# OpenSLAM-org/openslam_g2o

Hardware: AMD Instinct MI355X
Metric: linear-solve ms/iter (buildSystem + setLambda + solve + restoreDiagonal), 100k-pose BA (lower is better)
Workload: dtype f64; 1 GPU; synthetic BA (BASELINE.json configs[3]): 100000 poses / 1000000 landmarks / 5000000 observations, BlockSolver_6_3 semantics, Schur + multifrontal block Cholesky, lambda=10; poses=100000, landmarks=1000000, edges=5000000, parallelism=1 GPU, edge_data=estimates+measurements in HBM, errors/Jacobians evaluated inside buildSystem, information=identity, declared for the whole edge set (not read per edge)

## Files before the change

include/g2ohip.h:

```cpp
#ifndef G2OHIP_H
#define G2OHIP_H

#include <stddef.h>
#include <stdint.h>

#ifdef __cplusplus
extern "C" {
#endif

#define G2OHIP_OK 0
#define G2OHIP_NOT_PD 1
#define G2OHIP_REPEAT 2
#define G2OHIP_ERR_ARG (-1)
#define G2OHIP_ERR_HIP (-2)
#define G2OHIP_ERR_STATE (-3)
#define G2OHIP_ERR_UNSUPPORTED (-4)

#define G2OHIP_KERNEL_NONE 0
#define G2OHIP_KERNEL_HUBER 1
#define G2OHIP_KERNEL_PSEUDOHUBER 2
#define G2OHIP_KERNEL_CAUCHY 3
#define G2OHIP_KERNEL_SATURATED 4
#define G2OHIP_KERNEL_DCS 5

// ... 130 lines not shown
int g2ohip_solve_reduced(g2ohip_solver* s);
int g2ohip_solve_back_substitute(g2ohip_solver* s);

int g2ohip_host_register(g2ohip_solver* s, void* ptr, size_t bytes);
int g2ohip_host_unregister(g2ohip_solver* s, void* ptr);

int g2ohip_ba_set_edges(g2ohip_solver* s, int set, const int32_t* cam_vertex, const int32_t* point_vertex, const double* meas,
                        const double* info, double focal_length, double cx, double cy);
int g2ohip_ba_set_edges_classes(g2ohip_solver* s, int set, const int32_t* cam_vertex, const int32_t* point_vertex, const double* meas,
                                const double* info, int n_classes, const double* class_params, const int32_t* edge_class);
int g2ohip_ba_set_estimates(g2ohip_solver* s, int n_cams, const double* cams, const int32_t* cam_hidx, int n_points,
                            const double* points, const int32_t* point_hidx);
int g2ohip_ba_get_estimates(g2ohip_solver* s, double* cams, double* points);
int g2ohip_ba_get_estimates_of(g2ohip_solver* s, int n_cams, const int32_t* cam_index, double* cams, int n_points, const int32_t* point_index,
                               double* points);
int g2ohip_ba_fetch_estimates_begin(g2ohip_solver* s, double* cams, double* points, int point_pieces);
int g2ohip_ba_fetch_estimates_wait(g2ohip_solver* s, int piece);
int g2ohip_ba_linearize(g2ohip_solver* s, int jacobians);
int g2ohip_ba_update(g2ohip_solver* s);
int g2ohip_ba_push(g2ohip_solver* s);
int g2ohip_ba_pop(g2ohip_solver* s);
int g2ohip_ba_discard_top(g2ohip_solver* s);

int g2ohip_pg_set_edges(g2ohip_solver* s, int set, int type, const int32_t* vi, const int32_t* vj, const double* meas,
                        const double* info);
int g2ohip_pg_set_estimates(g2ohip_solver* s, int n_vertices, const double* poses, const int32_t* hidx);
int g2ohip_pg_get_estimates(g2ohip_solver* s, double* poses);
int g2ohip_pg_linearize(g2ohip_solver* s, int jacobians);
int g2ohip_pg_update(g2ohip_solver* s);
int g2ohip_pg_push(g2ohip_solver* s);
// ... 24 lines not shown
```

openslam_g2o_amd/capi.py:

```python
import ctypes as C
import os
import sys

import numpy as np

_HERE = os.path.dirname(os.path.abspath(__file__))
LIB_PATH = os.environ.get("G2OHIP_LIB") or os.path.join(_HERE, "lib", "libg2ohip.so")

c_int_p = C.POINTER(C.c_int32)
c_dbl_p = C.POINTER(C.c_double)

OK, NOT_PD, REPEAT = 0, 1, 2
ERR_UNSUPPORTED = -4
HPP, HPL, HLL, HSCHUR, DINV = 0, 1, 2, 3, 4
PART_NO_VERTEX0, PART_NO_VERTEX1, PART_NO_CHI2 = 1, 2, 4
ARR_BSCHUR, ARR_X, ARR_B, ARR_EXCHANGE, ARR_XP, ARR_XBOUNDARY, ARR_XHALO, ARR_SCHUR_DIAG = 100, 101, 102, 103, 104, 105, 106, 107
KERNEL_NONE, KERNEL_HUBER, KERNEL_PSEUDOHUBER, KERNEL_CAUCHY, KERNEL_SATURATED, KERNEL_DCS = 0, 1, 2, 3, 4, 5


class Stats(C.Structure):
    _fields_ = [(n, C.c_double) for n in (
        "timeQuadraticForm", "timeSchurComplement", "timeSymbolicDecomposition", "timeNumericDecomposition",
        "timeLinearSolution", "timeLinearSolver", "timeBackSubstitution")] + [(n, C.c_size_t) for n in (
            "hessianDimension", "hessianPoseDimension", "hessianLandmarkDimension", "choleskyNNZ", "numFronts",
# ... 2 lines not shown

    def as_dict(self):
        return {n: getattr(self, n) for n, _ in self._fields_}


EXPORTS = [
    "g2ohip_last_error", "g2ohip_device_count", "g2ohip_create", "g2ohip_destroy", "g2ohip_set_stream", "g2ohip_init",
    "g2ohip_add_edge_set", "g2ohip_build_structure", "g2ohip_set_edge_data", "g2ohip_set_edge_errors", "g2ohip_set_robust_kernel", "g2ohip_set_robust_kernel_per_edge",
    "g2ohip_build_system", "g2ohip_chi2", "g2ohip_set_lambda", "g2ohip_restore_diagonal", "g2ohip_max_diagonal",
    "g2ohip_compute_scale", "g2ohip_solve", "g2ohip_vector_size", "g2ohip_copy_x", "g2ohip_copy_b", "g2ohip_x_device",
    "g2ohip_b_device", "g2ohip_multiply_hessian", "g2ohip_sync", "g2ohip_set_profiling", "g2ohip_get_stats",
    "g2ohip_set_option", "g2ohip_get_nnzb", "g2ohip_get_pattern", "g2ohip_copy_values", "g2ohip_device_array",
    "g2ohip_solve_schur", "g2ohip_solve_reduced", "g2ohip_solve_back_substitute", "g2ohip_ls_create",
    "g2ohip_ls_destroy", "g2ohip_ls_init", "g2ohip_ls_solve", "g2ohip_ls_solve_pattern", "g2ohip_ls_get_stats", "g2ohip_ls_set_option",
    "g2ohip_kernel_slots", "g2ohip_kernel_name", "g2ohip_kernel_time", "g2ohip_add_schur_pattern", "g2ohip_set_edge_set_parts",
    "g2ohip_set_lambda_split", "g2ohip_host_register", "g2ohip_host_unregister", "g2ohip_ba_set_edges", "g2ohip_ba_set_edges_classes", "g2ohip_ba_set_estimates", "g2ohip_ba_get_estimates", "g2ohip_ba_get_estimates_of", "g2ohip_ba_fetch_estimates_begin", "g2ohip_ba_fetch_estimates_wait",
    "g2ohip_ba_linearize", "g2ohip_ba_update", "g2ohip_ba_push", "g2ohip_ba_pop", "g2ohip_ba_discard_top",
    "g2ohip_set_partition", "g2ohip_solve_reduced_local", "g2ohip_solve_reduced_shared", "g2ohip_solve_reduced_finish",
    "g2ohip_schur_operator_prepare", "g2ohip_schur_operator_apply", "g2ohip_solve_async", "g2ohip_trial_stats_begin", "g2ohip_trial_stats", "g2ohip_solve_reduced_finish_async", "g2ohip_exchange_setup", "g2ohip_exchange_pack", "g2ohip_exchange_unpack", "g2ohip_exchange_status",
    "g2ohip_get_partition", "g2ohip_partition_poses",
    "g2ohip_pg_set_edges", "g2ohip_pg_set_estimates", "g2ohip_pg_get_estimates", "g2ohip_pg_linearize", "g2ohip_pg_update",
    "g2ohip_pg_push", "g2ohip_pg_pop", "g2ohip_pg_discard_top", "g2ohip_copy_edge_data",
    "g2ohip_pg_set_landmark_edges", "g2ohip_pg_set_landmark_estimates", "g2ohip_pg_get_landmark_estimates",
    "g2ohip_compute_marginals", "g2ohip_set_x", "g2ohip_copy_diagonal",
    "g2ohip_comm_unique_id", "g2ohip_comm_init_rccl", "g2ohip_comm_init_host", "g2ohip_comm_init_peer", "g2ohip_comm_destroy", "g2ohip_comm_all_reduce",
    "g2ohip_update_structure", "g2ohip_clear_edge_sets", "g2ohip_solve_sharded", "g2ohip_chi2_sharded", "g2ohip_max_diagonal_sharded", "g2ohip_compute_scale_sharded",
]

HOST_ALLREDUCE_FN = C.CFUNCTYPE(C.c_int, C.c_void_p, C.POINTER(C.c_double), C.c_size_t, C.c_int)

_lib = None
# ... 61 lines not shown
    L.g2ohip_set_profiling.argtypes = [vp, C.c_int]
    L.g2ohip_get_stats.argtypes = [vp, C.POINTER(Stats)]
    L.g2ohip_set_option.argtypes = [vp, C.c_char_p, C.c_double]
    L.g2ohip_get_nnzb.argtypes = [vp, C.c_int, C.POINTER(C.c_int)]
    L.g2ohip_get_pattern.argtypes = [vp, C.c_int, c_int_p, c_int_p]
    L.g2ohip_copy_values.argtypes = [vp, C.c_int, c_dbl_p]
    L.g2ohip_device_array.argtypes = [vp, C.c_int, C.POINTER(vp), C.POINTER(C.c_size_t)]
    L.g2ohip_add_schur_pattern.argtypes = [vp, C.c_int, c_int_p, c_int_p]
    L.g2ohip_set_edge_set_parts.argtypes = [vp, C.c_int, C.c_int]
    L.g2ohip_set_lambda_split.argtypes = [vp, C.c_double, C.c_double, C.c_int]
    L.g2ohip_ba_set_edges.argtypes = [vp, C.c_int, c_int_p, c_int_p, c_dbl_p, c_dbl_p, C.c_double, C.c_double, C.c_double]
    L.g2ohip_ba_set_edges_classes.argtypes = [vp, C.c_int, c_int_p, c_int_p, c_dbl_p, c_dbl_p, C.c_int, c_dbl_p, c_int_p]
    L.g2ohip_ba_set_estimates.argtypes = [vp, C.c_int, c_dbl_p, c_int_p, C.c_int, c_dbl_p, c_int_p]
    L.g2ohip_ba_get_estimates.argtypes = [vp, c_dbl_p, c_dbl_p]
    L.g2ohip_ba_get_estimates_of.argtypes = [vp, C.c_int, c_int_p, c_dbl_p, C.c_int, c_int_p, c_dbl_p]
    L.g2ohip_set_edge_errors.argtypes = [vp, C.c_int, c_dbl_p]
    L.g2ohip_ba_fetch_estimates_begin.argtypes = [vp, c_dbl_p, c_dbl_p, C.c_int]
    L.g2ohip_ba_fetch_estimates_wait.argtypes = [vp, C.c_int]
    L.g2ohip_ba_linearize.argtypes = [vp, C.c_int]
    for n in ("g2ohip_ba_update", "g2ohip_ba_push", "g2ohip_ba_pop", "g2ohip_ba_discard_top", "g2ohip_pg_update", "g2ohip_pg_push",
              "g2ohip_pg_pop", "g2ohip_pg_discard_top"):
        getattr(L, n).argtypes = [vp]
    L.g2ohip_pg_set_edges.argtypes = [vp, C.c_int, C.c_int, c_int_p, c_int_p, c_dbl_p, c_dbl_p]
    L.g2ohip_pg_set_estimates.argtypes = [vp, C.c_int, c_dbl_p, c_int_p]
    L.g2ohip_pg_get_estimates.argtypes = [vp, c_dbl_p]
    L.g2ohip_pg_linearize.argtypes = [vp, C.c_int]
    L.g2ohip_pg_set_landmark_edges.argtypes = [vp, C.c_int, C.c_int, c_int_p, c_int_p, c_dbl_p, c_dbl_p, c_dbl_p]
    L.g2ohip_pg_set_landmark_estimates.argtypes = [vp, C.c_int, c_dbl_p, c_int_p]
    L.g2ohip_pg_get_landmark_estimates.argtypes = [vp, c_dbl_p]
    L.g2ohip_copy_edge_data.argtypes = [vp, C.c_int, c_dbl_p, c_dbl_p, c_dbl_p]
# ... 47 lines not shown
    return a.ctypes.data_as(c_dbl_p)


def _ptr(a):
    if a is None:
        return None, None
    if isinstance(a, np.ndarray):
        return C.c_void_p(a.ctypes.data), False
    if isinstance(a, int):
        return C.c_void_p(a), True
    if hasattr(a, "data_ptr"):
        return C.c_void_p(a.data_ptr()), bool(a.is_cuda)
    raise TypeError(type(a))


class HipBlockSolver:

    def __init__(self, pose_dim, landmark_dim, device=0):
        self.L = load()
        self.p, self.l = pose_dim, landmark_dim
        self.h = C.c_void_p()
        _check(self.L.g2ohip_create(C.byref(self.h), pose_dim, landmark_dim, device), "g2ohip_create")
        self._keep = {}
        self.nP = self.nL = 0

    def close(self):
        if getattr(self, "h", None) is not None and self.h.value:
            self.L.g2ohip_destroy(self.h)
            self.h = C.c_void_p()

# ... 317 lines not shown
        _check(self.L.g2ohip_ba_set_estimates(self.h, len(ch), _dp(cams), _ip(ch), len(ph), _dp(points), _ip(ph)),
               "baSetEstimates")

    def baGetEstimates(self):
        cams = np.empty((self._ba_n[0], 12))
        pts = np.empty((self._ba_n[1], 3))
        _check(self.L.g2ohip_ba_get_estimates(self.h, _dp(cams), _dp(pts)), "baGetEstimates")
        return cams, pts

    def baGetEstimatesOf(self, cam_index, point_index):
        ci, pi = _i32(cam_index), _i32(point_index)
        cams, pts = np.empty((len(ci), 12)), np.empty((len(pi), 3))
        _check(self.L.g2ohip_ba_get_estimates_of(self.h, len(ci), _ip(ci), _dp(cams), len(pi), _ip(pi), _dp(pts)), "baGetEstimatesOf")
        return cams, pts

    def baFetchEstimatesBegin(self, pieces=4):
        self._fetch = (np.empty((self._ba_n[0], 12)), np.empty((self._ba_n[1], 3)), pieces)
        _check(self.L.g2ohip_ba_fetch_estimates_begin(self.h, _dp(self._fetch[0]), _dp(self._fetch[1]), pieces), "baFetchEstimatesBegin")

    def baFetchEstimatesWait(self, piece):
        _check(self.L.g2ohip_ba_fetch_estimates_wait(self.h, piece), "baFetchEstimatesWait")
        return self._fetch[0], self._fetch[1]

    def baLinearize(self, jacobians=True):
        _check(self.L.g2ohip_ba_linearize(self.h, int(jacobians)), "baLinearize")

    def baUpdate(self):
        _check(self.L.g2ohip_ba_update(self.h), "baUpdate")

    def baPush(self):
# ... 183 lines not shown
```

openslam_g2o_amd/csrc/block_solver.h:

```cpp
#pragma once
#include <memory>

#include "common.h"
#include "comm.h"
#include "block_pcg.h"
#include "sparse_cholesky.h"

namespace g2ohip {

struct EdgeSet {
  int d = 0, n = 0, dim0 = 0, dim1 = 0;
  bool unary = false;
  int parts = 0;
  std::vector<int> v0, v1;
  int kernel_kind = 0;
  double delta = 1.0;
  DevBuf<double> rk;
  const double *J0 = nullptr, *J1 = nullptr, *omega = nullptr, *err = nullptr;
  DevBuf<double> own_J0, own_J1, own_omega, own_err;
  bool has_data = false;
  bool external = false;
  bool has_err = false;
  DevBuf<int> vp_ptr, vp_ent, vl_ptr, vl_ent;
  DevBuf<int> vp_act;
  int n_vp_act = 0;
  std::vector<int> h_vp_ent, h_vl_ent;
  std::vector<int> h_vl_ptr;
  DevBuf<int> op_dst, op_ptr, op_ent;
  DevBuf<int> ol_dst, ol_ptr, ol_ent;
  int n_op = 0, n_ol = 0;
  long n_vp_ent = 0, n_vl_ent = 0;
  bool touches_pose = false, touches_lm = false, first_pose = false, first_lm = false, first_op = false, first_ol = false;
};

struct SolverTimes {
  double quadratic = 0, schur = 0, numeric = 0, linsolve = 0, backsub = 0, residuals = 0, linearize = 0, update = 0;
};

class BlockSolver {
 public:
  BlockSolver(int p, int l, int device);
  ~BlockSolver();

  void init();
  void clear_edge_sets();
  int add_edge_set(int d, int n, const int* v0, const int* v1);
  void set_edge_set_parts(int set, int parts);
  void add_schur_pattern(int n, const int* rows, const int* cols);
  void build_structure(int nP, int nL, bool do_schur);
  bool update_structure(int new_poses, int set, int n, const int* v0, const int* v1);
  void set_edge_data(int set, const double* J0, const double* J1, const double* omega, const double* err, bool on_device);
  void set_edge_errors(int set, const double* err);
// ... 44 lines not shown
  void sync();
  void set_stream(hipStream_t st);
  hipStream_t stream() const { return st_; }

  int nnzb(int which) const;
  void get_pattern(int which, int* colptr, int* rowidx) const;
  void copy_values(int which, double* h);
  void device_array(int which, double** ptr, size_t* count);

  void ba_set_edges(int set, const int* cam_vertex, const int* point_vertex, const double* meas, const double* info, double f,
                    double cx, double cy);
  void ba_set_edges_classes(int set, const int* cam_vertex, const int* point_vertex, const double* meas, const double* info, double f,
                            double cx, double cy, int n_classes, const double* class_params, const int* edge_class);
  void ba_set_estimates(int n_cams, const double* cams, const int* cam_hidx, int n_points, const double* points, const int* point_hidx);
  void ba_get_estimates(double* cams, double* points);
  void ba_get_estimates_of(int n_cams, const int* cam_idx, double* cams, int n_points, const int* point_idx, double* points);
  void ba_fetch_begin(double* cams, double* points, int point_pieces);
  void ba_fetch_wait(int piece);
  static constexpr int kFetchMaxPieces = 17;
  void ba_linearize(bool jacobians);
  void ba_update();
  void ba_push();
  void ba_pop();
  void ba_discard_top();

  bool profiling = false;
  KernelProf prof;
  SolverTimes times;
  CholOptions chol_opt;
  size_t schur_tile_bytes = 39 * 1024;
// ... 180 lines not shown
    bool err_valid = false, jac_valid = false;
    DevBuf<double> chi_part;
    bool fused_ok = false;
    DevBuf<double> meas, cams, pts, cams_bak, pts_bak;
    DevBuf<double> meas_pm, omega_pm;
    DevBuf<int> pt_pm, cam_pm;
    DevBuf<double> meas_lm, omega_lm;
    DevBuf<int> cam_q, pt_q;
    DevBuf<double> meas_q, omega_q;
    DevBuf<int> cam_lm, pt_lm, hpl_lm, row_lm;
    DevBuf<int4> ll_rec;
    DevBuf<int> ll_edge;
    DevBuf<int> ll_row;
    DevBuf<double> ll_meas, ll_omega;
    DevBuf<int4> tile_ll;
    DevBuf<int> sel_idx;
    DevBuf<double> sel_out;
    bool ll_slots_ok = false;
    bool has_backup = false;
  } ba_;
  struct PgFrontEnd {
    int set = -1, type = 0, nv = 0;
    DevBuf<int> vi, vj, hidx;
    std::vector<int> h_vi, h_vj, h_hidx;
    DevBuf<double> meas, poses, poses_bak;
    bool has_backup = false;
    bool err_valid = false, jac_valid = false;
    int lm_set = -1, lm_type = 0, n_points = 0;
    DevBuf<int> vp, vl, pt_hidx;
    std::vector<int> h_vp, h_vl, h_pt_hidx;
// ... 10 lines not shown
```

openslam_g2o_amd/csrc/block_solver.hip:

```cpp
#include "block_solver.h"

#include <algorithm>
#include <atomic>
#include <chrono>
#include <cmath>
#include <cstring>
#include <numeric>

namespace g2ohip {

namespace {

constexpr int kThreads = 256;

template <int CTRL>
__device__ __forceinline__ double dpp_permute(double v) {
  const int lo = __double2loint(v), hi = __double2hiint(v);
  const int lo2 = __builtin_amdgcn_update_dpp(lo, lo, CTRL, 0xf, 0xf, true);
  const int hi2 = __builtin_amdgcn_update_dpp(hi, hi, CTRL, 0xf, 0xf, true);
  return __hiloint2double(hi2, lo2);
}
template <int G>
__device__ __forceinline__ double group_sum(double v) {
  if (G >= 2) v += dpp_permute<0xB1>(v);
// ... 1408 lines not shown
  if (!active || g >= 3) return;
  double cl[3];
#pragma unroll
  for (int j = 0; j < 3; ++j) cl[j] = c[j] + bl[(size_t)lm * 3 + j];
  const double* D = Dinv + (size_t)lm * 9;
  if (G == 1) {
#pragma unroll
    for (int i = 0; i < 3; ++i) xl[(size_t)lm * 3 + i] = D[i] * cl[0] + D[i + 3] * cl[1] + D[i + 6] * cl[2];
  } else {
    xl[(size_t)lm * 3 + g] = D[g] * cl[0] + D[g + 3] * cl[1] + D[g + 6] * cl[2];
  }
}

template <bool CLS>
__global__ void __launch_bounds__(kThreads) ba_back_substitute_slots_kernel(
    const int* __restrict__ tile_lm0, const int4* __restrict__ tile_ll, const int4* __restrict__ ll_rec, const int* __restrict__ ll_row,
    const double* __restrict__ ll_meas, const double* __restrict__ ll_omega, const double* __restrict__ cams,
    const double* __restrict__ pts, double f, double cx, double cy, int kind, double delta, int ident, const double* __restrict__ Dinv,
    const double* __restrict__ bl, const double* __restrict__ xp, double* __restrict__ xl, const double* __restrict__ ctab) {
  const int t = blockIdx.x, tid = threadIdx.x, NT = blockDim.x;
  const int l0 = tile_lm0[(size_t)t * 8];
  const int4 tl = tile_ll[t];
  for (int sb = 0; sb < tl.y; sb += NT) {
    const int si = sb + tid;
    const size_t sg = (size_t)tl.x + min(si, tl.y - 1);
    int4 rc = ll_rec[sg];
    if (si >= tl.y) rc.x = (int)0x80000fffu;
    const int ent = rc.x;
    const int krel = ent & 0xfff, K = (ent >> 12) & 0xff, lmi = (ent >> 20) & 0x7ff;
    const bool head = ent >= 0;
    const int pos = head ? 0 : lmi;
    const int row = krel != 0xfff ? ll_row[sg] : -1;
    double c[3] = {0.0, 0.0, 0.0};
    {
      double T[12], X[3], z2[2], Op[4], xv[6];
      const double* Xp = pts + (size_t)rc.z * 3;
      X[0] = Xp[0]; X[1] = Xp[1]; X[2] = Xp[2];
      load_vec<12>(cams + (size_t)ba_edge_class<CLS>(rc.y, ctab, f, cx, cy, kind, delta) * 12, T);
      load_vec<2>(ll_meas + sg * 2, z2);
      load_vec<6>(xp + (size_t)max(row, 0) * 6, xv);
      if (ident) {
        Op[0] = Op[3] = 1.0;
        Op[1] = Op[2] = 0.0;
      } else {
        load_vec<4>(ll_omega + sg * 4, Op);
      }
      if (row >= 0) {
        BaEdgeLin L;
        ba_edge_linearize(T, X, z2, Op, f, cx, cy, kind, delta, true, L);
        double t0 = 0.0, t1 = 0.0;
#pragma unroll
        for (int a = 0; a < 6; ++a) {
          t0 += L.B[0 + 2 * a] * xv[a];
          t1 += L.B[1 + 2 * a] * xv[a];
        }
        const double w = L.w;
        const double u0 = w * (L.O[0] * t0 + L.O[2] * t1), u1 = w * (L.O[1] * t0 + L.O[3] * t1);
#pragma unroll
        for (int j = 0; j < 3; ++j) c[j] = -(L.A[0 + 2 * j] * u0 + L.A[1 + 2 * j] * u1);
      }
    }
    for (int d = 1; d < tl.w; d <<= 1) {
      const bool take = pos + d < K;
#pragma unroll
      for (int i = 0; i < 3; ++i) {
        const double o = __shfl_down(c[i], d);
        if (take) c[i] += o;
      }
    }
    if (head) {
      const int lm = l0 + lmi;
      double cl[3];
#pragma unroll
      for (int j = 0; j < 3; ++j) cl[j] = c[j] + bl[(size_t)lm * 3 + j];
      const double* D = Dinv + (size_t)lm * 9;
#pragma unroll
      for (int i = 0; i < 3; ++i) xl[(size_t)lm * 3 + i] = D[i] * cl[0] + D[i + 3] * cl[1] + D[i + 6] * cl[2];
    }
  }
}

#ifndef G2OHIP_ASMP_OCC
#define G2OHIP_ASMP_OCC 2
#endif
template <int G, bool CLS = false>
__global__ void __launch_bounds__(kThreads, G2OHIP_ASMP_OCC) ba_assemble_poses_kernel(
    int nP, const int* __restrict__ vptr, const double* __restrict__ cams, const double* __restrict__ pts,
    const int* __restrict__ cam_pm, const int* __restrict__ pt_pm, const double* __restrict__ meas_pm, const double* __restrict__ omega_pm,
    double f, double cx, double cy, int kind, double delta, double* __restrict__ Hpp, const int* __restrict__ diag_blk,
    double* __restrict__ bp, int accumulate, int ident, const int* __restrict__ act, const double* __restrict__ ctab) {
  const int gt = blockIdx.x * blockDim.x + threadIdx.x;
  const int vi_ = gt / G, g = gt % G;
  const bool active = vi_ < nP;
// ... 2431 lines not shown

void BlockSolver::solve_back_substitute() {
  require_structure();
  if (!schur_) return;
  G2OHIP_HIP_CHECK(hipSetDevice(device_));
  solve_back_substitute_impl();
}

void BlockSolver::solve_back_substitute_impl() {
  if (profiling) tb_.start(st_);
  const size_t sizeP = (size_t)nP_ * p_;
  prof.begin(KernelProf::kBackSub, st_);
  if (ba_recompute_ok()) {
    EdgeSet& es = *sets_[ba_.set];
    const int GL = ba_lm_group();
    if (ba_fuse_landmarks && ba_.ll_slots_ok && n_tiles_ > 0) {
#define G2OHIP_BA_BACK_SLOTS(CC)                                                                                                   \
  hipLaunchKernelGGL((ba_back_substitute_slots_kernel<CC>), dim3(n_tiles_), dim3(kThreads), 0, st_, d_tile_lm0.p, ba_.tile_ll.p,    \
                     ba_.ll_rec.p, ba_.ll_row.p, ba_.ll_meas.p, ba_.ll_omega.p, ba_.cams.p, ba_.pts.p, ba_.f, ba_.cx, ba_.cy,       \
                     es.kernel_kind, es.delta, ba_.omega_identity ? 1 : 0, d_Dinv.p, d_b.p + sizeP, d_x.p, d_x.p + sizeP, ba_.ctab.p)
      if (ba_.n_classes > 1) G2OHIP_BA_BACK_SLOTS(true);
      else G2OHIP_BA_BACK_SLOTS(false);
#undef G2OHIP_BA_BACK_SLOTS
    } else
#define G2OHIP_BA_BACK(GG) G2OHIP_BA_BACK_(GG, false)
#define G2OHIP_BA_BACK_(GG, CC)                                                                                                    \
  hipLaunchKernelGGL((ba_back_substitute_kernel<GG, CC>), dim3(grid_for((size_t)nL_ * GG)), dim3(kThreads), 0, st_, nL_, es.vl_ptr.p, \
                     ba_.cams.p, ba_.pts.p, ba_.cam_lm.p, ba_.pt_lm.p, ba_.meas_lm.p, ba_.omega_lm.p, ba_.row_lm.p, ba_.f,          \
                     ba_.cx, ba_.cy, es.kernel_kind, es.delta, ba_.omega_identity ? 1 : 0, d_Dinv.p, d_b.p + sizeP, d_x.p,           \
                     d_x.p + sizeP, ba_.ctab.p)
    if (ba_.n_classes > 1) G2OHIP_BA_BACK_(8, true);
    else if (GL == 1) G2OHIP_BA_BACK(1);
    else if (GL == 4) G2OHIP_BA_BACK(4);
    else G2OHIP_BA_BACK(8);
#undef G2OHIP_BA_BACK
// ... 441 lines not shown
  const size_t k = (size_t)blockIdx.x * blockDim.x + threadIdx.x;
  if (k >= n) return;
  const size_t e = (size_t)(ent[k] >> 1);
  cam_o[k] = cam_v[e];
  pt_o[k] = pt_v[e];
  meas_o[2 * k] = meas[2 * e];
  meas_o[2 * k + 1] = meas[2 * e + 1];
  if (omega_o)
    for (int i = 0; i < 4; ++i) omega_o[4 * k + i] = omega[4 * e + i];
  if (hpl_o) {
    const int h = edge_hpl[e];
    hpl_o[k] = h;
    row_o[k] = h >= 0 ? v1[e] : -1;
  }
}
__global__ void ba_gather_slots_kernel(const int4* __restrict__ tile_ll, const int* __restrict__ slots, const int* __restrict__ vl_ent,
                                       const int* __restrict__ cam_lm, const int* __restrict__ pt_lm, const int* __restrict__ hpl_lm,
                                       const int* __restrict__ row_lm, const double* __restrict__ meas_lm, const double* __restrict__ omega_lm,
                                       int4* __restrict__ rec, int* __restrict__ edge, int* __restrict__ srow, double* __restrict__ ms,
                                       double* __restrict__ os) {
  const int4 tl = tile_ll[blockIdx.x];
  for (int i = threadIdx.x; i < tl.y; i += blockDim.x) {
    const size_t sidx = (size_t)tl.x + i;
    const int w = slots[sidx];
    int4 r = make_int4(w, 0, 0, -1);
    int ed = 0, row = -1;
    double m0 = 0.0, m1 = 0.0, o[4] = {0.0, 0.0, 0.0, 0.0};
    if ((w & 0xfff) != 0xfff) {
      const size_t k = (size_t)tl.z + (w & 0xfff);
      r = make_int4(w, cam_lm[k], pt_lm[k], hpl_lm[k]);
// ... 140 lines not shown
    ba_.meas_lm.alloc(std::max<size_t>(nl * 2, 1));
    ba_.cam_lm.alloc(std::max<size_t>(nl, 1));
    ba_.pt_lm.alloc(std::max<size_t>(nl, 1));
    ba_.hpl_lm.alloc(std::max<size_t>(nl, 1));
    ba_.row_lm.alloc(std::max<size_t>(nl, 1));
    if (d_omega) ba_.omega_lm.alloc(std::max<size_t>(nl * 4, 1));
    if (nl)
      hipLaunchKernelGGL(ba_gather_lists_kernel, dim3(grid_for(nl)), dim3(kThreads), 0, st_, nl, es.vl_ent.p, ba_.cam_v.p, ba_.pt_v.p, ba_.meas.p,
                         d_omega, ba_.edge_hpl.p, d_v1.p, ba_.cam_lm.p, ba_.pt_lm.p, ba_.meas_lm.p,
                         d_omega ? ba_.omega_lm.p : (double*)nullptr, ba_.hpl_lm.p, ba_.row_lm.p);
    G2OHIP_HIP_CHECK(hipGetLastError());
    lap("pose-major + landmark-major copies");
    ba_.ll_slots_ok = false;
    if (schur_ && n_tiles_ > 0 && tiles_cover_all_ && n_split_tiles_ == 0 && (int)tile_lm0_h_.size() == n_tiles_ + 1 &&
        (int)es.h_vl_ptr.size() == nL_ + 1) {
      constexpr int kIdleSlot = (int)0x80000fffu;
      std::vector<int4> tl((size_t)n_tiles_);
      std::vector<int> cnt((size_t)n_tiles_, 0);
      std::atomic<bool> okf(true);
      auto walk = [&](int t, int* out, int& kmax) {
        const int l0 = tile_lm0_h_[t], l1 = tile_lm0_h_[t + 1];
        const int kb = es.h_vl_ptr[l0];
        int used = 0, total = 0;
        kmax = 0;
        for (int lm = l0; lm < l1; ++lm) {
          const int K = es.h_vl_ptr[lm + 1] - es.h_vl_ptr[lm], lmi = lm - l0;
          if (K > 64 || lmi >= 0x7ff || es.h_vl_ptr[lm + 1] - kb >= 0xfff) return -1;
          const int need = std::max(K, 1);
          if (used + need > 64) {
            if (out)
              for (int i = used; i < 64; ++i) out[total + i - used] = kIdleSlot;
            total += 64 - used;
            used = 0;
          }
          if (out) {
            if (K == 0) out[total] = 0xfff | (lmi << 20);
            for (int j = 0; j < K; ++j)
              out[total + j] = (es.h_vl_ptr[lm] + j - kb) | (K << 12) | (j == 0 ? (lmi << 20) : (int)(0x80000000u | ((unsigned)j << 20)));
          }
          total += need;
          used = (used + need) & 63;
          kmax = std::max(kmax, K);
        }
        if (used) {
          if (out)
            for (int i = used; i < 64; ++i) out[total + i - used] = kIdleSlot;
          total += 64 - used;
        }
        return total;
      };
      host_parallel_for((size_t)n_tiles_, [&](size_t t0_, size_t t1_) {
        for (size_t t = t0_; t < t1_; ++t) {
          int kmax = 0;
          const int c = walk((int)t, nullptr, kmax);
          if (c < 0) okf.store(false);
          cnt[t] = std::max(c, 0);
        }
      }, 64);
      size_t ns = 0;
      for (int t = 0; t < n_tiles_; ++t) {
        tl[t].x = (int)ns;
        ns += (size_t)cnt[t];
      }
      if (okf.load() && ns < ((size_t)1 << 31)) {
        std::vector<int> slots(std::max<size_t>(ns, 1), kIdleSlot);
        host_parallel_for((size_t)n_tiles_, [&](size_t t0_, size_t t1_) {
          for (size_t t = t0_; t < t1_; ++t) {
            int kmax = 0;
            walk((int)t, slots.data() + tl[t].x, kmax);
            tl[t] = make_int4(tl[t].x, cnt[t], es.h_vl_ptr[tile_lm0_h_[t]], kmax);
          }
        }, 64);
        const size_t nsa = slots.size();
        DevBuf<int> d_slots;
        d_slots.upload(slots, st_);
        ba_.tile_ll.upload(tl, st_);
        ba_.ll_rec.alloc(nsa);
        ba_.ll_edge.alloc(nsa);
        ba_.ll_row.alloc(nsa);
        ba_.ll_meas.alloc(nsa * 2);
        if (d_omega) ba_.ll_omega.alloc(nsa * 4);
        if (ns == 0) {
          const int4 idle = make_int4(kIdleSlot, 0, 0, -1);
          const int none = -1;
          ba_.ll_rec.upload(&idle, 1, st_);
          ba_.ll_row.upload(&none, 1, st_);
          ba_.ll_edge.zero(st_);
          ba_.ll_meas.zero(st_);
        } else {
          hipLaunchKernelGGL(ba_gather_slots_kernel, dim3(n_tiles_), dim3(kThreads), 0, st_, ba_.tile_ll.p, d_slots.p, es.vl_ent.p, ba_.cam_lm.p,
                             ba_.pt_lm.p, ba_.hpl_lm.p, ba_.row_lm.p, ba_.meas_lm.p, d_omega ? ba_.omega_lm.p : (const double*)nullptr,
// ... 6 lines not shown
    }
    lap("lane slots of the tiles");
    G2OHIP_HIP_CHECK(hipStreamSynchronize(st_));
  }
  lap("pose-major / landmark-major uploads");
  if (!(ba_fused && ba_.fused_ok)) {
    es.own_J0.alloc(n * 6);
    es.own_J1.alloc(n * 12);
  }
  es.own_err.alloc(n * 2);
  es.J0 = es.own_J0.p; es.J1 = es.own_J1.p; es.omega = es.own_omega.p; es.err = es.own_err.p;
  es.has_data = false;
  prepare_ba_tile_kernels();
  G2OHIP_HIP_CHECK(hipStreamSynchronize(st_));
  lap("buffers, kernel attributes, sync");
}

bool BlockSolver::ba_recompute_ok() const {
  if (!schur_ || p_ != 6 || l_ != 3 || ba_.set < 0 || !ba_fused || !ba_.fused_ok || ba_.n_cams <= 0) return false;
  if (ba_.sys_version < 0 || ba_.sys_version != ba_.est_version) return false;
  const EdgeSet& bs = *sets_[ba_.set];
  if (bs.kernel_kind != ba_.sys_kind || bs.delta != ba_.sys_delta) return false;
  for (size_t i = 0; i < sets_.size(); ++i)
    if ((int)i != ba_.set && sets_[i]->n > 0 && sets_[i]->touches_lm) return false;
  return true;
}

void BlockSolver::ba_validate() {
  if (ba_.set < 0 || ba_.h_cam_v.empty() || ba_.h_cam_hidx.empty()) return;
  ba_validate_edges(*sets_[ba_.set], ba_.h_cam_v.data(), ba_.h_pt_v.data(), ba_.h_cam_v.size());
// ... 643 lines not shown
```

openslam_g2o_amd/csrc/capi.hip:

```cpp
#include "../../include/g2ohip.h"

#include <cstdlib>
#include <cstring>
#include <string>

#include "block_solver.h"

namespace g2ohip {
std::string& last_error_ref() {
  static thread_local std::string e;
  return e;
}
}

using namespace g2ohip;

struct g2ohip_solver {
  std::unique_ptr<BlockSolver> impl;
};

struct g2ohip_linear_solver {
  int bs = 0, device = 0;
  hipStream_t st = nullptr;
  std::unique_ptr<SparseCholesky> chol;
// ... 631 lines not shown
int g2ohip_ba_get_estimates(g2ohip_solver* s, double* cams, double* points) {
  REQUIRE_HANDLE(s);
  return guarded([&] {
    s->impl->ba_get_estimates(cams, points);
    return G2OHIP_OK;
  });
}
int g2ohip_ba_get_estimates_of(g2ohip_solver* s, int n_cams, const int32_t* cam_index, double* cams, int n_points, const int32_t* point_index,
                               double* points) {
  REQUIRE_HANDLE(s);
  return guarded([&] {
    s->impl->ba_get_estimates_of(n_cams, cam_index, cams, n_points, point_index, points);
    return G2OHIP_OK;
  });
}
int g2ohip_ba_fetch_estimates_begin(g2ohip_solver* s, double* cams, double* points, int point_pieces) {
  REQUIRE_HANDLE(s);
  return guarded([&] {
    s->impl->ba_fetch_begin(cams, points, point_pieces);
    return G2OHIP_OK;
  });
}
int g2ohip_ba_fetch_estimates_wait(g2ohip_solver* s, int piece) {
  REQUIRE_HANDLE(s);
  return guarded([&] {
    s->impl->ba_fetch_wait(piece);
    return G2OHIP_OK;
  });
}
int g2ohip_ba_linearize(g2ohip_solver* s, int jacobians) {
// ... 356 lines not shown
```

Before: 1.141 ms/iter.

## Run landmark back-substitution as persistent 64-lane groups with prefetch

```diff
diff --git a/include/g2ohip.h b/include/g2ohip.h
--- a/include/g2ohip.h
+++ b/include/g2ohip.h
@@ -168,6 +168,10 @@
 int g2ohip_ba_get_estimates(g2ohip_solver* s, double* cams, double* points);
 int g2ohip_ba_get_estimates_of(g2ohip_solver* s, int n_cams, const int32_t* cam_index, double* cams, int n_points, const int32_t* point_index,
                                double* points);
+int g2ohip_ba_plan_lane_slots(int n_tiles, const int32_t* tile_lm0, const int32_t* list_ptr, long long* n_slots, int32_t* tile_ll,
+                              int32_t* group_ll, int32_t* slot_words);
+int g2ohip_ba_get_lane_slots(g2ohip_solver* s, int* n_tiles, long long* n_slots, int32_t* tile_lm0, int32_t* tile_ll, int32_t* group_ll,
+                             int32_t* slot_words);
 int g2ohip_ba_fetch_estimates_begin(g2ohip_solver* s, double* cams, double* points, int point_pieces);
 int g2ohip_ba_fetch_estimates_wait(g2ohip_solver* s, int piece);
 int g2ohip_ba_linearize(g2ohip_solver* s, int jacobians);
diff --git a/openslam_g2o_amd/capi.py b/openslam_g2o_amd/capi.py
--- a/openslam_g2o_amd/capi.py
+++ b/openslam_g2o_amd/capi.py
@@ -40,7 +40,7 @@
     "g2ohip_solve_schur", "g2ohip_solve_reduced", "g2ohip_solve_back_substitute", "g2ohip_ls_create",
     "g2ohip_ls_destroy", "g2ohip_ls_init", "g2ohip_ls_solve", "g2ohip_ls_solve_pattern", "g2ohip_ls_get_stats", "g2ohip_ls_set_option",
     "g2ohip_kernel_slots", "g2ohip_kernel_name", "g2ohip_kernel_time", "g2ohip_add_schur_pattern", "g2ohip_set_edge_set_parts",
-    "g2ohip_set_lambda_split", "g2ohip_host_register", "g2ohip_host_unregister", "g2ohip_ba_set_edges", "g2ohip_ba_set_edges_classes", "g2ohip_ba_set_estimates", "g2ohip_ba_get_estimates", "g2ohip_ba_get_estimates_of", "g2ohip_ba_fetch_estimates_begin", "g2ohip_ba_fetch_estimates_wait",
+    "g2ohip_set_lambda_split", "g2ohip_host_register", "g2ohip_host_unregister", "g2ohip_ba_set_edges", "g2ohip_ba_set_edges_classes", "g2ohip_ba_set_estimates", "g2ohip_ba_get_estimates", "g2ohip_ba_get_estimates_of", "g2ohip_ba_plan_lane_slots", "g2ohip_ba_get_lane_slots", "g2ohip_ba_fetch_estimates_begin", "g2ohip_ba_fetch_estimates_wait",
     "g2ohip_ba_linearize", "g2ohip_ba_update", "g2ohip_ba_push", "g2ohip_ba_pop", "g2ohip_ba_discard_top",
     "g2ohip_set_partition", "g2ohip_solve_reduced_local", "g2ohip_solve_reduced_shared", "g2ohip_solve_reduced_finish",
     "g2ohip_schur_operator_prepare", "g2ohip_schur_operator_apply", "g2ohip_solve_async", "g2ohip_trial_stats_begin", "g2ohip_trial_stats", "g2ohip_solve_reduced_finish_async", "g2ohip_exchange_setup", "g2ohip_exchange_pack", "g2ohip_exchange_unpack", "g2ohip_exchange_status",
@@ -132,6 +132,8 @@
     L.g2ohip_ba_set_estimates.argtypes = [vp, C.c_int, c_dbl_p, c_int_p, C.c_int, c_dbl_p, c_int_p]
     L.g2ohip_ba_get_estimates.argtypes = [vp, c_dbl_p, c_dbl_p]
     L.g2ohip_ba_get_estimates_of.argtypes = [vp, C.c_int, c_int_p, c_dbl_p, C.c_int, c_int_p, c_dbl_p]
+    L.g2ohip_ba_plan_lane_slots.argtypes = [C.c_int, c_int_p, c_int_p, C.POINTER(C.c_longlong), c_int_p, c_int_p, c_int_p]
+    L.g2ohip_ba_get_lane_slots.argtypes = [vp, C.POINTER(C.c_int), C.POINTER(C.c_longlong), c_int_p, c_int_p, c_int_p, c_int_p]
     L.g2ohip_set_edge_errors.argtypes = [vp, C.c_int, c_dbl_p]
     L.g2ohip_ba_fetch_estimates_begin.argtypes = [vp, c_dbl_p, c_dbl_p, C.c_int]
     L.g2ohip_ba_fetch_estimates_wait.argtypes = [vp, C.c_int]
@@ -209,6 +211,20 @@
     raise TypeError(type(a))
 
 
+def plan_lane_slots(tile_lm0, list_ptr):
+    L = load()
+    tl0, lp = _i32(tile_lm0), _i32(list_ptr)
+    nt, ns = len(tl0) - 1, C.c_longlong()
+    _check(L.g2ohip_ba_plan_lane_slots(nt, _ip(tl0), _ip(lp), C.byref(ns), None, None, None), "plan_lane_slots")
+    if ns.value < 0:
+        return None
+    t = dict(tile_ll=np.zeros((nt, 4), dtype=np.int32), group_ll=np.zeros((ns.value // 64, 2), dtype=np.int32),
+             slot_words=np.zeros(ns.value, dtype=np.int32))
+    _check(L.g2ohip_ba_plan_lane_slots(nt, _ip(tl0), _ip(lp), C.byref(ns), _ip(t["tile_ll"]), _ip(t["group_ll"]), _ip(t["slot_words"])),
+           "plan_lane_slots")
+    return t
+
+
 class HipBlockSolver:
 
     def __init__(self, pose_dim, landmark_dim, device=0):
@@ -556,6 +572,15 @@
         _check(self.L.g2ohip_ba_get_estimates_of(self.h, len(ci), _ip(ci), _dp(cams), len(pi), _ip(pi), _dp(pts)), "baGetEstimatesOf")
         return cams, pts
 
+    def baLaneSlots(self):
+        nt, ns = C.c_int(), C.c_longlong()
+        _check(self.L.g2ohip_ba_get_lane_slots(self.h, C.byref(nt), C.byref(ns), None, None, None, None), "baLaneSlots")
+        t = dict(tile_lm0=np.zeros(nt.value + 1, dtype=np.int32), tile_ll=np.zeros((nt.value, 4), dtype=np.int32),
+                 group_ll=np.zeros((ns.value // 64, 2), dtype=np.int32), slot_words=np.zeros(ns.value, dtype=np.int32))
+        _check(self.L.g2ohip_ba_get_lane_slots(self.h, None, None, _ip(t["tile_lm0"]), _ip(t["tile_ll"]), _ip(t["group_ll"]),
+                                               _ip(t["slot_words"])), "baLaneSlots")
+        return t
+
     def baFetchEstimatesBegin(self, pieces=4):
         self._fetch = (np.empty((self._ba_n[0], 12)), np.empty((self._ba_n[1], 3)), pieces)
         _check(self.L.g2ohip_ba_fetch_estimates_begin(self.h, _dp(self._fetch[0]), _dp(self._fetch[1]), pieces), "baFetchEstimatesBegin")
diff --git a/openslam_g2o_amd/csrc/block_solver.h b/openslam_g2o_amd/csrc/block_solver.h
--- a/openslam_g2o_amd/csrc/block_solver.h
+++ b/openslam_g2o_amd/csrc/block_solver.h
@@ -36,6 +36,13 @@
 struct SolverTimes {
   double quadratic = 0, schur = 0, numeric = 0, linsolve = 0, backsub = 0, residuals = 0, linearize = 0, update = 0;
 };
+
+struct BaLaneSlots {
+  std::vector<int4> tile_ll;
+  std::vector<int> slots;
+  std::vector<int2> group_ll;
+};
+bool ba_plan_lane_slots(int n_tiles, const int* tile_lm0, const int* vl_ptr, BaLaneSlots& out);
 
 class BlockSolver {
  public:
@@ -110,6 +117,7 @@
                             double cx, double cy, int n_classes, const double* class_params, const int* edge_class);
   void ba_set_estimates(int n_cams, const double* cams, const int* cam_hidx, int n_points, const double* points, const int* point_hidx);
   void ba_get_estimates(double* cams, double* points);
+  void ba_get_lane_slots(int* n_tiles, long long* n_slots, int* tile_lm0, int* tile_ll, int* group_ll, int* slot_words);
   void ba_get_estimates_of(int n_cams, const int* cam_idx, double* cams, int n_points, const int* point_idx, double* points);
   void ba_fetch_begin(double* cams, double* points, int point_pieces);
   void ba_fetch_wait(int piece);
@@ -320,6 +328,11 @@
     DevBuf<int> ll_row;
     DevBuf<double> ll_meas, ll_omega;
     DevBuf<int4> tile_ll;
+    DevBuf<int2> group_ll;
+    int n_groups = 0;
+    int back_wg_per_cu[2] = {1, 1};
+    std::vector<int4> h_tile_ll;
+    std::vector<int2> h_group_ll;
     DevBuf<int> sel_idx;
     DevBuf<double> sel_out;
     bool ll_slots_ok = false;
diff --git a/openslam_g2o_amd/csrc/block_solver.hip b/openslam_g2o_amd/csrc/block_solver.hip
--- a/openslam_g2o_amd/csrc/block_solver.hip
+++ b/openslam_g2o_amd/csrc/block_solver.hip
@@ -1446,53 +1446,67 @@
 
 template <bool CLS>
 __global__ void __launch_bounds__(kThreads) ba_back_substitute_slots_kernel(
-    const int* __restrict__ tile_lm0, const int4* __restrict__ tile_ll, const int4* __restrict__ ll_rec, const int* __restrict__ ll_row,
+    int n_groups, const int2* __restrict__ group_ll, const int4* __restrict__ ll_rec, const int* __restrict__ ll_row,
     const double* __restrict__ ll_meas, const double* __restrict__ ll_omega, const double* __restrict__ cams,
     const double* __restrict__ pts, double f, double cx, double cy, int kind, double delta, int ident, const double* __restrict__ Dinv,
     const double* __restrict__ bl, const double* __restrict__ xp, double* __restrict__ xl, const double* __restrict__ ctab) {
-  const int t = blockIdx.x, tid = threadIdx.x, NT = blockDim.x;
-  const int l0 = tile_lm0[(size_t)t * 8];
-  const int4 tl = tile_ll[t];
-  for (int sb = 0; sb < tl.y; sb += NT) {
-    const int si = sb + tid;
-    const size_t sg = (size_t)tl.x + min(si, tl.y - 1);
-    int4 rc = ll_rec[sg];
-    if (si >= tl.y) rc.x = (int)0x80000fffu;
+  const int lane = threadIdx.x & 63, wpb = blockDim.x >> 6;
+  const int stride = gridDim.x * wpb;
+  int g = blockIdx.x * wpb + (threadIdx.x >> 6);
+  if (g >= n_groups) return;
+  size_t sg = (size_t)g * 64 + lane;
+  int4 rc = ll_rec[sg];
+  int row = ll_row[sg];
+  double z2[2];
+  load_vec<2>(ll_meas + sg * 2, z2);
+  int2 gl = group_ll[g];
+  for (;;) {
     const int ent = rc.x;
     const int krel = ent & 0xfff, K = (ent >> 12) & 0xff, lmi = (ent >> 20) & 0x7ff;
     const bool head = ent >= 0;
     const int pos = head ? 0 : lmi;
-    const int row = krel != 0xfff ? ll_row[sg] : -1;
+    if (krel == 0xfff) row = -1;
+    double T[12], X[3], Op[4], xv[6], blv[3], D[9];
+    const double* Xp = pts + (size_t)rc.z * 3;
+    X[0] = Xp[0]; X[1] = Xp[1]; X[2] = Xp[2];
+    load_vec<12>(cams + (size_t)ba_edge_class<CLS>(rc.y, ctab, f, cx, cy, kind, delta) * 12, T);
+    load_vec<6>(xp + (size_t)max(row, 0) * 6, xv);
+    if (ident) {
+      Op[0] = Op[3] = 1.0;
+      Op[1] = Op[2] = 0.0;
+    } else {
+      load_vec<4>(ll_omega + sg * 4, Op);
+    }
+    const int lm = gl.x + (head ? lmi : 0);
+#pragma unroll
+    for (int j = 0; j < 3; ++j) blv[j] = bl[(size_t)lm * 3 + j];
+#pragma unroll
+    for (int j = 0; j < 9; ++j) D[j] = Dinv[(size_t)lm * 9 + j];
+    const int gn = g + stride;
+    const bool more = gn < n_groups;
+    const int gq = more ? gn : g;
+    const size_t sn = (size_t)gq * 64 + lane;
+    const int4 rcn = ll_rec[sn];
+    const int rown = ll_row[sn];
+    double zn[2];
+    load_vec<2>(ll_meas + sn * 2, zn);
+    const int2 gln = group_ll[gq];
     double c[3] = {0.0, 0.0, 0.0};
-    {
-      double T[12], X[3], z2[2], Op[4], xv[6];
-      const double* Xp = pts + (size_t)rc.z * 3;
-      X[0] = Xp[0]; X[1] = Xp[1]; X[2] = Xp[2];
-      load_vec<12>(cams + (size_t)ba_edge_class<CLS>(rc.y, ctab, f, cx, cy, kind, delta) * 12, T);
-      load_vec<2>(ll_meas + sg * 2, z2);
-      load_vec<6>(xp + (size_t)max(row, 0) * 6, xv);
-      if (ident) {
-        Op[0] = Op[3] = 1.0;
-        Op[1] = Op[2] = 0.0;
-      } else {
-        load_vec<4>(ll_omega + sg * 4, Op);
+    if (row >= 0) {
+      BaEdgeLin L;
+      ba_edge_linearize(T, X, z2, Op, f, cx, cy, kind, delta, true, L);
+      double t0 = 0.0, t1 = 0.0;
+#pragma unroll
+      for (int a = 0; a < 6; ++a) {
+        t0 += L.B[0 + 2 * a] * xv[a];
+        t1 += L.B[1 + 2 * a] * xv[a];
       }
-      if (row >= 0) {
-        BaEdgeLin L;
-        ba_edge_linearize(T, X, z2, Op, f, cx, cy, kind, delta, true, L);
-        double t0 = 0.0, t1 = 0.0;
-#pragma unroll
-        for (int a = 0; a < 6; ++a) {
-          t0 += L.B[0 + 2 * a] * xv[a];
-          t1 += L.B[1 + 2 * a] * xv[a];
-        }
-        const double w = L.w;
-        const double u0 = w * (L.O[0] * t0 + L.O[2] * t1), u1 = w * (L.O[1] * t0 + L.O[3] * t1);
-#pragma unroll
-        for (int j = 0; j < 3; ++j) c[j] = -(L.A[0 + 2 * j] * u0 + L.A[1 + 2 * j] * u1);
-      }
-    }
-    for (int d = 1; d < tl.w; d <<= 1) {
+      const double w = L.w;
+      const double u0 = w * (L.O[0] * t0 + L.O[2] * t1), u1 = w * (L.O[1] * t0 + L.O[3] * t1);
+#pragma unroll
+      for (int j = 0; j < 3; ++j) c[j] = -(L.A[0 + 2 * j] * u0 + L.A[1 + 2 * j] * u1);
+    }
+    for (int d = 1; d < gl.y; d <<= 1) {
       const bool take = pos + d < K;
 #pragma unroll
       for (int i = 0; i < 3; ++i) {
@@ -1501,14 +1515,19 @@
       }
     }
     if (head) {
-      const int lm = l0 + lmi;
       double cl[3];
 #pragma unroll
-      for (int j = 0; j < 3; ++j) cl[j] = c[j] + bl[(size_t)lm * 3 + j];
-      const double* D = Dinv + (size_t)lm * 9;
+      for (int j = 0; j < 3; ++j) cl[j] = c[j] + blv[j];
 #pragma unroll
       for (int i = 0; i < 3; ++i) xl[(size_t)lm * 3 + i] = D[i] * cl[0] + D[i + 3] * cl[1] + D[i + 6] * cl[2];
     }
+    if (!more) break;
+    g = gn;
+    sg = sn;
+    rc = rcn;
+    row = rown;
+    z2[0] = zn[0]; z2[1] = zn[1];
+    gl = gln;
   }
 }
 
@@ -3970,11 +3989,13 @@
   if (ba_recompute_ok()) {
     EdgeSet& es = *sets_[ba_.set];
     const int GL = ba_lm_group();
-    if (ba_fuse_landmarks && ba_.ll_slots_ok && n_tiles_ > 0) {
+    if (ba_fuse_landmarks && ba_.ll_slots_ok && ba_.n_groups > 0) {
 #define G2OHIP_BA_BACK_SLOTS(CC)                                                                                                   \
-  hipLaunchKernelGGL((ba_back_substitute_slots_kernel<CC>), dim3(n_tiles_), dim3(kThreads), 0, st_, d_tile_lm0.p, ba_.tile_ll.p,    \
-                     ba_.ll_rec.p, ba_.ll_row.p, ba_.ll_meas.p, ba_.ll_omega.p, ba_.cams.p, ba_.pts.p, ba_.f, ba_.cx, ba_.cy,       \
-                     es.kernel_kind, es.delta, ba_.omega_identity ? 1 : 0, d_Dinv.p, d_b.p + sizeP, d_x.p, d_x.p + sizeP, ba_.ctab.p)
+  hipLaunchKernelGGL((ba_back_substitute_slots_kernel<CC>),                                                                        \
+                     dim3(std::min((ba_.n_groups + kThreads / 64 - 1) / (kThreads / 64), num_cus_ * ba_.back_wg_per_cu[CC])),      \
+                     dim3(kThreads), 0, st_, ba_.n_groups, ba_.group_ll.p, ba_.ll_rec.p, ba_.ll_row.p, ba_.ll_meas.p,               \
+                     ba_.ll_omega.p, ba_.cams.p, ba_.pts.p, ba_.f, ba_.cx, ba_.cy, es.kernel_kind, es.delta,                       \
+                     ba_.omega_identity ? 1 : 0, d_Dinv.p, d_b.p + sizeP, d_x.p, d_x.p + sizeP, ba_.ctab.p)
       if (ba_.n_classes > 1) G2OHIP_BA_BACK_SLOTS(true);
       else G2OHIP_BA_BACK_SLOTS(false);
 #undef G2OHIP_BA_BACK_SLOTS
@@ -4446,6 +4467,79 @@
     row_o[k] = h >= 0 ? v1[e] : -1;
   }
 }
+bool ba_plan_lane_slots(int n_tiles, const int* tile_lm0, const int* vl_ptr, BaLaneSlots& out) {
+  constexpr int kIdleSlot = (int)0x80000fffu;
+  std::vector<int4>& tl = out.tile_ll;
+  tl.assign((size_t)n_tiles, make_int4(0, 0, 0, 0));
+  out.slots.clear();
+  out.group_ll.clear();
+  std::vector<int> cnt((size_t)n_tiles, 0);
+  std::atomic<bool> okf(true);
+  auto walk = [&](int t, int* slot_out, int& kmax) {
+    const int l0 = tile_lm0[t], l1 = tile_lm0[t + 1];
+    const int kb = vl_ptr[l0];
+    int used = 0, total = 0;
+    kmax = 0;
+    for (int lm = l0; lm < l1; ++lm) {
+      const int K = vl_ptr[lm + 1] - vl_ptr[lm], lmi = lm - l0;
+      if (K > 64 || lmi >= 0x7ff || vl_ptr[lm + 1] - kb >= 0xfff) return -1;
+      const int need = std::max(K, 1);
+      if (used + need > 64) {
+        if (slot_out)
+          for (int i = used; i < 64; ++i) slot_out[total + i - used] = kIdleSlot;
+        total += 64 - used;
+        used = 0;
+      }
+      if (slot_out) {
+        if (K == 0) slot_out[total] = 0xfff | (lmi << 20);
+        for (int j = 0; j < K; ++j)
+          slot_out[total + j] = (vl_ptr[lm] + j - kb) | (K << 12) | (j == 0 ? (lmi << 20) : (int)(0x80000000u | ((unsigned)j << 20)));
+      }
+      total += need;
+      used = (used + need) & 63;
+      kmax = std::max(kmax, K);
+    }
+    if (used) {
+      if (slot_out)
+        for (int i = used; i < 64; ++i) slot_out[total + i - used] = kIdleSlot;
+      total += 64 - used;
+    }
+    return total;
+  };
+  host_parallel_for((size_t)n_tiles, [&](size_t t0_, size_t t1_) {
+    for (size_t t = t0_; t < t1_; ++t) {
+      int kmax = 0;
+      const int c = walk((int)t, nullptr, kmax);
+      if (c < 0) okf.store(false);
+      cnt[t] = std::max(c, 0);
+    }
+  }, 64);
+  size_t ns = 0;
+  for (int t = 0; t < n_tiles; ++t) {
+    tl[t].x = (int)ns;
+    ns += (size_t)cnt[t];
+  }
+  if (!okf.load() || ns >= ((size_t)1 << 31)) return false;
+  out.slots.assign(std::max<size_t>(ns, 1), kIdleSlot);
+  out.group_ll.assign(ns / 64, make_int2(0, 0));
+  host_parallel_for((size_t)n_tiles, [&](size_t t0_, size_t t1_) {
+    for (size_t t = t0_; t < t1_; ++t) {
+      int kmax = 0;
+      int* sl = out.slots.data() + tl[t].x;
+      walk((int)t, sl, kmax);
+      tl[t] = make_int4(tl[t].x, cnt[t], vl_ptr[tile_lm0[t]], kmax);
+      for (int g0 = 0; g0 < cnt[t]; g0 += 64) {
+        int kg = 0;
+        for (int i = 0; i < 64; ++i) kg = std::max(kg, (sl[g0 + i] >> 12) & 0xff);
+        if (kg > kmax) okf.store(false);
+        out.group_ll[(size_t)(tl[t].x + g0) / 64] = make_int2(tile_lm0[t], kg);
+      }
+    }
+  }, 64);
+  if (!okf.load()) throw ArgFailure("lane slots: a group's longest list exceeds its tile's");
+  return true;
+}
+
 __global__ void ba_gather_slots_kernel(const int4* __restrict__ tile_ll, const int* __restrict__ slots, const int* __restrict__ vl_ent,
                                        const int* __restrict__ cam_lm, const int* __restrict__ pt_lm, const int* __restrict__ hpl_lm,
                                        const int* __restrict__ row_lm, const double* __restrict__ meas_lm, const double* __restrict__ omega_lm,
@@ -4616,67 +4710,26 @@
     ba_.ll_slots_ok = false;
     if (schur_ && n_tiles_ > 0 && tiles_cover_all_ && n_split_tiles_ == 0 && (int)tile_lm0_h_.size() == n_tiles_ + 1 &&
         (int)es.h_vl_ptr.size() == nL_ + 1) {
-      constexpr int kIdleSlot = (int)0x80000fffu;
-      std::vector<int4> tl((size_t)n_tiles_);
-      std::vector<int> cnt((size_t)n_tiles_, 0);
-      std::atomic<bool> okf(true);
-      auto walk = [&](int t, int* out, int& kmax) {
-        const int l0 = tile_lm0_h_[t], l1 = tile_lm0_h_[t + 1];
-        const int kb = es.h_vl_ptr[l0];
-        int used = 0, total = 0;
-        kmax = 0;
-        for (int lm = l0; lm < l1; ++lm) {
-          const int K = es.h_vl_ptr[lm + 1] - es.h_vl_ptr[lm], lmi = lm - l0;
-          if (K > 64 || lmi >= 0x7ff || es.h_vl_ptr[lm + 1] - kb >= 0xfff) return -1;
-          const int need = std::max(K, 1);
-          if (used + need > 64) {
-            if (out)
-              for (int i = used; i < 64; ++i) out[total + i - used] = kIdleSlot;
-            total += 64 - used;
-            used = 0;
-          }
-          if (out) {
-            if (K == 0) out[total] = 0xfff | (lmi << 20);
-            for (int j = 0; j < K; ++j)
-              out[total + j] = (es.h_vl_ptr[lm] + j - kb) | (K << 12) | (j == 0 ? (lmi << 20) : (int)(0x80000000u | ((unsigned)j << 20)));
-          }
-          total += need;
-          used = (used + need) & 63;
-          kmax = std::max(kmax, K);
-        }
-        if (used) {
-          if (out)
-            for (int i = used; i < 64; ++i) out[total + i - used] = kIdleSlot;
-          total += 64 - used;
-        }
-        return total;
-      };
-      host_parallel_for((size_t)n_tiles_, [&](size_t t0_, size_t t1_) {
-        for (size_t t = t0_; t < t1_; ++t) {
-          int kmax = 0;
-          const int c = walk((int)t, nullptr, kmax);
-          if (c < 0) okf.store(false);
-          cnt[t] = std::max(c, 0);
-        }
-      }, 64);
-      size_t ns = 0;
-      for (int t = 0; t < n_tiles_; ++t) {
-        tl[t].x = (int)ns;
-        ns += (size_t)cnt[t];
-      }
-      if (okf.load() && ns < ((size_t)1 << 31)) {
-        std::vector<int> slots(std::max<size_t>(ns, 1), kIdleSlot);
-        host_parallel_for((size_t)n_tiles_, [&](size_t t0_, size_t t1_) {
-          for (size_t t = t0_; t < t1_; ++t) {
-            int kmax = 0;
-            walk((int)t, slots.data() + tl[t].x, kmax);
-            tl[t] = make_int4(tl[t].x, cnt[t], es.h_vl_ptr[tile_lm0_h_[t]], kmax);
-          }
-        }, 64);
+      BaLaneSlots ls;
+      if (ba_plan_lane_slots(n_tiles_, tile_lm0_h_.data(), es.h_vl_ptr.data(), ls)) {
+        const std::vector<int>& slots = ls.slots;
+        const std::vector<int4>& tl = ls.tile_ll;
+        const size_t ns = (size_t)ls.group_ll.size() * 64;
+        constexpr int kIdleSlot = (int)0x80000fffu;
         const size_t nsa = slots.size();
         DevBuf<int> d_slots;
         d_slots.upload(slots, st_);
         ba_.tile_ll.upload(tl, st_);
+        ba_.group_ll.upload(ls.group_ll, st_);
+        ba_.n_groups = (int)ls.group_ll.size();
+        ba_.h_tile_ll = tl;
+        ba_.h_group_ll = ls.group_ll;
+        for (int cc = 0; cc < 2; ++cc) {
+          int nb = 0;
+          G2OHIP_HIP_CHECK(hipOccupancyMaxActiveBlocksPerMultiprocessor(
+              &nb, cc ? (const void*)ba_back_substitute_slots_kernel<true> : (const void*)ba_back_substitute_slots_kernel<false>, kThreads, 0));
+          ba_.back_wg_per_cu[cc] = std::max(nb, 1);
+        }
         ba_.ll_rec.alloc(nsa);
         ba_.ll_edge.alloc(nsa);
         ba_.ll_row.alloc(nsa);
@@ -4713,6 +4766,22 @@
   prepare_ba_tile_kernels();
   G2OHIP_HIP_CHECK(hipStreamSynchronize(st_));
   lap("buffers, kernel attributes, sync");
+}
+
+void BlockSolver::ba_get_lane_slots(int* n_tiles, long long* n_slots, int* tile_lm0, int* tile_ll, int* group_ll, int* slot_words) {
+  if (ba_.set < 0 || !ba_.ll_slots_ok) throw StateFailure("ba_get_lane_slots: the set has no lane slots (see g2ohip_ba_plan_lane_slots)");
+  G2OHIP_HIP_CHECK(hipSetDevice(device_));
+  const size_t ns = (size_t)ba_.n_groups * 64;
+  if (n_tiles) *n_tiles = n_tiles_;
+  if (n_slots) *n_slots = (long long)ns;
+  if (tile_lm0) std::copy(tile_lm0_h_.begin(), tile_lm0_h_.end(), tile_lm0);
+  if (tile_ll) std::memcpy(tile_ll, ba_.h_tile_ll.data(), ba_.h_tile_ll.size() * sizeof(int4));
+  if (group_ll) std::memcpy(group_ll, ba_.h_group_ll.data(), ba_.h_group_ll.size() * sizeof(int2));
+  if (slot_words && ns) {
+    std::vector<int4> rec(ns);
+    ba_.ll_rec.download(rec.data(), ns, st_);
+    for (size_t i = 0; i < ns; ++i) slot_words[i] = rec[i].x;
+  }
 }
 
 bool BlockSolver::ba_recompute_ok() const {
diff --git a/openslam_g2o_amd/csrc/capi.hip b/openslam_g2o_amd/csrc/capi.hip
--- a/openslam_g2o_amd/csrc/capi.hip
+++ b/openslam_g2o_amd/csrc/capi.hip
@@ -669,6 +669,31 @@
     return G2OHIP_OK;
   });
 }
+int g2ohip_ba_plan_lane_slots(int n_tiles, const int32_t* tile_lm0, const int32_t* list_ptr, long long* n_slots, int32_t* tile_ll,
+                              int32_t* group_ll, int32_t* slot_words) {
+  return guarded([&] {
+    if (n_tiles < 0 || !tile_lm0 || !list_ptr || !n_slots) throw ArgFailure("ba_plan_lane_slots: null array");
+    BaLaneSlots ls;
+    if (!ba_plan_lane_slots(n_tiles, tile_lm0, list_ptr, ls)) {
+      *n_slots = -1;
+      return G2OHIP_OK;
+    }
+    const size_t ns = ls.group_ll.size() * 64;
+    *n_slots = (long long)ns;
+    if (tile_ll) std::memcpy(tile_ll, ls.tile_ll.data(), ls.tile_ll.size() * sizeof(int4));
+    if (group_ll) std::memcpy(group_ll, ls.group_ll.data(), ls.group_ll.size() * sizeof(int2));
+    if (slot_words) std::memcpy(slot_words, ls.slots.data(), ns * sizeof(int));
+    return G2OHIP_OK;
+  });
+}
+int g2ohip_ba_get_lane_slots(g2ohip_solver* s, int* n_tiles, long long* n_slots, int32_t* tile_lm0, int32_t* tile_ll, int32_t* group_ll,
+                             int32_t* slot_words) {
+  REQUIRE_HANDLE(s);
+  return guarded([&] {
+    s->impl->ba_get_lane_slots(n_tiles, n_slots, tile_lm0, tile_ll, group_ll, slot_words);
+    return G2OHIP_OK;
+  });
+}
 int g2ohip_ba_fetch_estimates_begin(g2ohip_solver* s, double* cams, double* points, int point_pieces) {
   REQUIRE_HANDLE(s);
   return guarded([&] {
```

Measured after the change: 1.133 ms/iter, median of 6. Within noise of the previous version (-0.7%).
